# ErickRosete/tacorl

Hardware: NVIDIA B200
Metric: play_lmp_train_frames_per_sec (higher is better)
Workload: dtype bf16

## Files before the change

tacorl_b200/csrc/conv_tc.cu:

```cuda
#include "common.cuh"
#include "internal.h"
#include <cuda.h>
#include <cuda_bf16.h>
#include <algorithm>

namespace tacorl {

constexpr int CV_MAXT = 16;
constexpr int CV_STAGES = 8;
constexpr int CV_THREADS = 192;

struct ConvGeom {
  int BW, BH;
  int tiles_x, tiles_y, num_tiles;
  int ntaps;
  int tap_x[CV_MAXT], tap_p[CV_MAXT], tap_y[CV_MAXT];
  int RA, RB;
  int OH, OW, oys, oy0, oxs, ox0;
};

struct ConvEpi {
  const float* bias;
  int relu;
  const __nv_bfloat16* gate;
  __nv_bfloat16* out_bf16;
  float* out_f32;
};

__device__ __forceinline__ uint32_t cv_smem(const void* p) { return (uint32_t)__cvta_generic_to_shared(p); }
__device__ __forceinline__ void cv_mbar_init(uint32_t bar, uint32_t count) {
  asm volatile("mbarrier.init.shared::cta.b64 [%0], %1;" ::"r"(bar), "r"(count));
}
__device__ __forceinline__ void cv_mbar_expect_tx(uint32_t bar, uint32_t bytes) {
  asm volatile("mbarrier.arrive.expect_tx.shared::cta.b64 _, [%0], %1;" ::"r"(bar), "r"(bytes) : "memory");
}
__device__ __forceinline__ void cv_mbar_arrive(uint32_t bar) {
  asm volatile("mbarrier.arrive.shared::cta.b64 _, [%0];" ::"r"(bar) : "memory");
}
__device__ __forceinline__ void cv_mbar_wait(uint32_t bar, uint32_t parity) {
  uint32_t done;
  do {
    asm volatile(
        "{\n\t.reg .pred p;\n\t"
        "mbarrier.try_wait.parity.shared::cta.b64 p, [%1], %2;\n\t"
        "selp.u32 %0, 1, 0, p;\n\t}"
        : "=r"(done) : "r"(bar), "r"(parity) : "memory");
  } while (!done);
}
__device__ __forceinline__ void cv_tma_2d(uint32_t dst, const CUtensorMap* tm, int c0, int c1, uint32_t bar) {
  asm volatile(
      "cp.async.bulk.tensor.2d.shared::cluster.global.mbarrier::complete_tx::bytes [%0], [%1, {%2, %3}], [%4];"
      ::"r"(dst), "l"(tm), "r"(c0), "r"(c1), "r"(bar) : "memory");
}
__device__ __forceinline__ void cv_tma_4d(uint32_t dst, const CUtensorMap* tm, int c0, int c1, int c2, int c3, uint32_t bar) {
  asm volatile(
      "cp.async.bulk.tensor.4d.shared::cluster.global.mbarrier::complete_tx::bytes [%0], [%1, {%2, %3, %4, %5}], [%6];"
      ::"r"(dst), "l"(tm), "r"(c0), "r"(c1), "r"(c2), "r"(c3), "r"(bar) : "memory");
}
__device__ __forceinline__ void cv_tma_5d(uint32_t dst, const CUtensorMap* tm, int c0, int c1, int c2, int c3, int c4,
                                          uint32_t bar) {
  asm volatile(
      "cp.async.bulk.tensor.5d.shared::cluster.global.mbarrier::complete_tx::bytes [%0], [%1, {%2, %3, %4, %5, %6}], [%7];"
      ::"r"(dst), "l"(tm), "r"(c0), "r"(c1), "r"(c2), "r"(c3), "r"(c4), "r"(bar) : "memory");
}
__device__ __forceinline__ void cv_cp16(uint32_t dst, const void* src, uint32_t src_bytes) {
  asm volatile("cp.async.cg.shared.global [%0], [%1], 16, %2;" ::"r"(dst), "l"(src), "r"(src_bytes) : "memory");
}
__device__ __forceinline__ void cv_cp_async_arrive(uint32_t bar) {
  asm volatile("cp.async.mbarrier.arrive.noinc.shared::cta.b64 [%0];" ::"r"(bar) : "memory");
}
__device__ __forceinline__ void cv_st32(void* p, const uint32_t (&v)[8]) {
  asm volatile("st.global.v8.b32 [%0], {%1,%2,%3,%4,%5,%6,%7,%8};"
               ::"l"(p), "r"(v[0]), "r"(v[1]), "r"(v[2]), "r"(v[3]), "r"(v[4]), "r"(v[5]), "r"(v[6]), "r"(v[7]) : "memory");
}
__device__ __forceinline__ void cv_commit_group() { asm volatile("cp.async.commit_group;" ::: "memory"); }
template <int N> __device__ __forceinline__ void cv_wait_group() {
  asm volatile("cp.async.wait_group %0;" ::"n"(N) : "memory");
}
__device__ __forceinline__ void cv_wait_group_dyn(int n) {
  switch (n) {
    case 0: cv_wait_group<0>(); break;
    case 1: cv_wait_group<1>(); break;
    case 2: cv_wait_group<2>(); break;
    case 3: cv_wait_group<3>(); break;
    default: cv_wait_group<4>(); break;
  }
}
__device__ __forceinline__ void cv_fence_async() { asm volatile("fence.proxy.async.shared::cta;" ::: "memory"); }
__device__ __forceinline__ void cv_fence_before() { asm volatile("tcgen05.fence::before_thread_sync;" ::: "memory"); }
__device__ __forceinline__ void cv_fence_after() { asm volatile("tcgen05.fence::after_thread_sync;" ::: "memory"); }
__device__ __forceinline__ void cv_commit(uint32_t bar) {
  asm volatile("tcgen05.commit.cta_group::1.mbarrier::arrive::one.shared::cluster.b64 [%0];" ::"r"(bar) : "memory");
}
__device__ __forceinline__ void cv_mma(uint32_t tmem_d, uint64_t adesc, uint64_t bdesc, uint32_t idesc, uint32_t acc) {
  asm volatile(
      "{\n\t.reg .pred p;\n\t"
      "setp.ne.b32 p, %4, 0;\n\t"
      "tcgen05.mma.cta_group::1.kind::f16 [%0], %1, %2, %3, p;\n\t}"
      ::"r"(tmem_d), "l"(adesc), "l"(bdesc), "r"(idesc), "r"(acc) : "memory");
}
__device__ __forceinline__ void cv_ld16(uint32_t taddr, uint32_t (&r)[16]) {
  asm volatile(
      "tcgen05.ld.sync.aligned.32x32b.x16.b32 {%0,%1,%2,%3,%4,%5,%6,%7,%8,%9,%10,%11,%12,%13,%14,%15}, [%16];"
      : "=r"(r[0]), "=r"(r[1]), "=r"(r[2]), "=r"(r[3]), "=r"(r[4]), "=r"(r[5]), "=r"(r[6]), "=r"(r[7]),
        "=r"(r[8]), "=r"(r[9]), "=r"(r[10]), "=r"(r[11]), "=r"(r[12]), "=r"(r[13]), "=r"(r[14]), "=r"(r[15])
      : "r"(taddr));
  asm volatile("tcgen05.wait::ld.sync.aligned;" ::: "memory");
}
__device__ __forceinline__ void cv_ld16_nowait(uint32_t taddr, uint32_t (&r)[16]) {
  asm volatile(
      "tcgen05.ld.sync.aligned.32x32b.x16.b32 {%0,%1,%2,%3,%4,%5,%6,%7,%8,%9,%10,%11,%12,%13,%14,%15}, [%16];"
      : "=r"(r[0]), "=r"(r[1]), "=r"(r[2]), "=r"(r[3]), "=r"(r[4]), "=r"(r[5]), "=r"(r[6]), "=r"(r[7]),
        "=r"(r[8]), "=r"(r[9]), "=r"(r[10]), "=r"(r[11]), "=r"(r[12]), "=r"(r[13]), "=r"(r[14]), "=r"(r[15])
      : "r"(taddr));
}
__device__ __forceinline__ void cv_ld_wait() { asm volatile("tcgen05.wait::ld.sync.aligned;" ::: "memory"); }
__device__ __forceinline__ uint64_t cv_desc(uint32_t saddr, uint32_t lbo, uint32_t sbo) {
  uint64_t d = 0;
  d |= (uint64_t)((saddr >> 4) & 0x3FFF);
  d |= (uint64_t)((lbo >> 4) & 0x3FFF) << 16;
  d |= (uint64_t)((sbo >> 4) & 0x3FFF) << 32;
  d |= (uint64_t)1 << 46;
  d |= (uint64_t)2 << 61;
  return d;
}

// ... 37 lines not shown
  __syncthreads();
  cv_fence_after();
  const uint32_t tmem_base = *tmem_slot;

  if (warp == 0) {
    if (lane == 0) {
      cv_mbar_expect_tx(w_bar, g.ntaps * W_TAP_BYTES);
      for (int t = 0; t < g.ntaps; ++t) cv_tma_2d(w_base + t * W_TAP_BYTES, &tmW, 0, t * BN, w_bar);
      const uint32_t box_bytes = (uint32_t)(g.BW * g.BH) * 128;
      uint32_t it = 0;
      for (int tile = blockIdx.x; tile < g.num_tiles; tile += gridDim.x) {
        const int n = tile / tiles_per_frame, rem = tile - n * tiles_per_frame;
        const int ty = rem / g.tiles_x, tx = rem - ty * g.tiles_x;
        const int x0 = tx * g.BW, y0 = ty * g.BH;
        for (int t = 0; t < g.ntaps; ++t, ++it) {
          const int s = it % CV_STAGES;
          cv_mbar_wait(empty_bar(s), ((it / CV_STAGES) & 1) ^ 1);
          cv_mbar_expect_tx(full_bar(s), box_bytes);
          cv_tma_5d(a_base + s * A_BYTES, &tmA, 0, x0 + g.tap_x[t], g.tap_p[t], y0 + g.tap_y[t], n, full_bar(s));
        }
      }
    }
  } else if (warp == 1) {
    if (lane == 0) {
      cv_mbar_wait(w_bar, 0);
      const uint32_t idesc = (1u << 4) | (1u << 7) | (1u << 10) | ((uint32_t)(BN >> 3) << 17) | ((uint32_t)(128 >> 4) << 24);
      uint64_t bdesc[NTAPS * 4];
#pragma unroll
      for (int i = 0; i < NTAPS * 4; ++i) bdesc[i] = cv_desc(w_base + (i >> 2) * W_TAP_BYTES + (i & 3) * 32, 16, 1024);
      const uint64_t adesc0 = cv_desc(a_base, 16, 1024);
      uint32_t it = 0, lt = 0;
      for (int tile = blockIdx.x; tile < g.num_tiles; tile += gridDim.x, ++lt) {
        const uint32_t acc = lt & 1;
        cv_mbar_wait(tempty_bar(acc), ((lt >> 1) & 1) ^ 1);
        cv_fence_after();
        const uint32_t tmem_d = tmem_base + acc * ACC_COLS;
#pragma unroll
        for (int t = 0; t < NTAPS; ++t, ++it) {
          const int s = it % CV_STAGES;
          cv_mbar_wait(full_bar(s), (it / CV_STAGES) & 1);
          cv_fence_after();
          const uint64_t adesc = adesc0 + (uint64_t)(s * (A_BYTES >> 4));
#pragma unroll
          for (int k = 0; k < 4; ++k) cv_mma(tmem_d, adesc + 2 * k, bdesc[t * 4 + k], idesc, (t > 0 || k > 0) ? 1u : 0u);
          cv_commit(empty_bar(s));
        }
        cv_commit(tfull_bar(acc));
      }
    }
  } else {
    const int q = warp & 3;
    const int r = q * 32 + lane;
    const int a_l = r / g.BW, b_l = r - a_l * g.BW;
    uint32_t lt = 0;
    for (int tile = blockIdx.x; tile < g.num_tiles; tile += gridDim.x, ++lt) {
      const uint32_t acc = lt & 1;
      const int n = tile / tiles_per_frame, rem = tile - n * tiles_per_frame;
      const int ty = rem / g.tiles_x, tx = rem - ty * g.tiles_x;
      const int a = ty * g.BH + a_l, b = tx * g.BW + b_l;
      const bool row_ok = a_l < g.BH && a < g.RA && b < g.RB;
      const long long opix = row_ok ? ((long long)n * g.OH + (a * g.oys + g.oy0)) * g.OW + (b * g.oxs + g.ox0) : 0;
      uint4 gate[BN / 8];
      if (ep.gate && row_ok) {
        const uint4* gp = reinterpret_cast<const uint4*>(ep.gate + opix * BN);
#pragma unroll
        for (int j = 0; j < BN / 8; ++j) gate[j] = __ldg(gp + j);
      }
      cv_mbar_wait(tfull_bar(acc), (lt >> 1) & 1);
      cv_fence_after();
#pragma unroll
      for (int c0 = 0; c0 < BN; c0 += 16) {
        uint32_t rr[16];
        cv_ld16(tmem_base + acc * ACC_COLS + ((uint32_t)(q * 32) << 16) + c0, rr);
        if (!row_ok) continue;
        float v[16];
#pragma unroll
        for (int j = 0; j < 16; ++j) v[j] = __uint_as_float(rr[j]) + s_bias[c0 + j];
        if (ep.relu) {
#pragma unroll
          for (int j = 0; j < 16; ++j) v[j] = fmaxf(v[j], 0.f);
        }
        if (ep.gate) {
          const uint4 g0 = gate[c0 / 8], g1 = gate[c0 / 8 + 1];
          const __nv_bfloat162* h0 = reinterpret_cast<const __nv_bfloat162*>(&g0);
          const __nv_bfloat162* h1 = reinterpret_cast<const __nv_bfloat162*>(&g1);
#pragma unroll
          for (int j = 0; j < 4; ++j) {
            const float2 f0 = __bfloat1622float2(h0[j]), f1 = __bfloat1622float2(h1[j]);
            if (f0.x <= 0.f) v[2 * j] = 0.f;
            if (f0.y <= 0.f) v[2 * j + 1] = 0.f;
            if (f1.x <= 0.f) v[8 + 2 * j] = 0.f;
            if (f1.y <= 0.f) v[8 + 2 * j + 1] = 0.f;
          }
        }
        if (ep.out_bf16) {
          uint32_t pk[8];
#pragma unroll
          for (int j = 0; j < 8; ++j) {
            __nv_bfloat162 t2 = __floats2bfloat162_rn(v[2 * j], v[2 * j + 1]);
            pk[j] = *reinterpret_cast<uint32_t*>(&t2);
          }
          cv_st32(ep.out_bf16 + opix * BN + c0, pk);
        }
        if (ep.out_f32) {
          uint32_t lo[8], hi[8];
#pragma unroll
          for (int j = 0; j < 8; ++j) { lo[j] = __float_as_uint(v[j]); hi[j] = __float_as_uint(v[8 + j]); }
          cv_st32(ep.out_f32 + opix * BN + c0, lo);
          cv_st32(ep.out_f32 + opix * BN + c0 + 8, hi);
        }
      }
      cv_fence_before();
      __syncwarp();
      if (lane == 0) cv_mbar_arrive(tempty_bar(acc));
    }
  }
  cv_fence_before();
  __syncthreads();
  if (warp == 1) {
    cv_fence_after();
    asm volatile("tcgen05.dealloc.cta_group::1.sync.aligned.b32 %0, %1;" ::"r"(tmem_base), "r"(TMEM_COLS) : "memory");
  }
}

struct ConvLinGeom {
  int W, OH, OW;
  int frame_rows;
  int tiles_per_frame, num_tiles;
  int ntaps, load_rows;
  int stages;
  int shift[CV_MAXT];
  int OHt, OWt, oys, oy0, oxs, ox0;
};
constexpr int CL_MAX_STAGES = 8;

template <int BN, int NTAPS, int KSTEPS>
__global__ void __launch_bounds__(CV_THREADS, 1)
conv_lin_kernel(const __grid_constant__ ConvLinGeom g, const __grid_constant__ CUtensorMap tmA,
                const __grid_constant__ CUtensorMap tmW, const ConvEpi ep) {
  constexpr uint32_t W_TAP_BYTES = BN * 128;
  constexpr uint32_t ACC_COLS = BN < 32 ? 32 : BN;
  constexpr int NACC = 4;
  constexpr uint32_t TMEM_COLS = NACC * ACC_COLS;
  extern __shared__ __align__(1024) uint8_t smem_raw[];
  uint8_t* smem = (uint8_t*)(((uintptr_t)smem_raw + 1023) & ~(uintptr_t)1023);
  const uint32_t stage_bytes = ((uint32_t)g.load_rows * 128 + 1023) & ~1023u;
  const uint32_t w_base = cv_smem(smem);
  const uint32_t a_base = w_base + g.ntaps * W_TAP_BYTES;
  uint64_t* bars = (uint64_t*)(smem + g.ntaps * W_TAP_BYTES + g.stages * stage_bytes);
  const int CL_STAGES = g.stages;
  uint32_t* tmem_slot = (uint32_t*)(bars + 2 * CL_MAX_STAGES + 2 * NACC + 1);
  auto full_bar = [&](int s) { return cv_smem(bars + s); };
  auto empty_bar = [&](int s) { return cv_smem(bars + CL_MAX_STAGES + s); };
  auto tfull_bar = [&](int a) { return cv_smem(bars + 2 * CL_MAX_STAGES + a); };
  auto tempty_bar = [&](int a) { return cv_smem(bars + 2 * CL_MAX_STAGES + NACC + a); };
  const uint32_t w_bar = cv_smem(bars + 2 * CL_MAX_STAGES + 2 * NACC);
  const int warp = threadIdx.x >> 5, lane = threadIdx.x & 31;
  __shared__ float s_bias[BN];
  if (threadIdx.x < BN) s_bias[threadIdx.x] = ep.bias ? ep.bias[threadIdx.x] : 0.f;

  if (threadIdx.x == 0) {
    for (int s = 0; s < CL_STAGES; ++s) { cv_mbar_init(full_bar(s), 1); cv_mbar_init(empty_bar(s), 1); }
    for (int a = 0; a < NACC; ++a) { cv_mbar_init(tfull_bar(a), 1); cv_mbar_init(tempty_bar(a), 4); }
    cv_mbar_init(w_bar, 1);
    asm volatile("fence.mbarrier_init.release.cluster;" ::: "memory");
  }
  if (warp == 1) {
// ... 166 lines not shown
  __syncthreads();
  cv_fence_after();
  const uint32_t tmem_base = *tmem_slot;

  if (warp == 0) {
    if (lane == 0) {
      cv_mbar_expect_tx(w_bar, 4 * W_TAP_BYTES);
      for (int t = 0; t < 4; ++t) cv_tma_2d(w_base + t * W_TAP_BYTES, &tmW, 0, t * 128, w_bar);
      uint32_t it = 0;
      for (int tile = blockIdx.x; tile < g.num_tiles; tile += gridDim.x, ++it) {
        const int n = tile / tiles_per_frame, rem = tile - n * tiles_per_frame;
        const int ty = rem / g.tiles_x, tx = rem - ty * g.tiles_x;
        const int s = it % DG_STAGES;
        cv_mbar_wait(empty_bar(s), ((it / DG_STAGES) & 1) ^ 1);
        cv_mbar_expect_tx(full_bar(s), A_BYTES);
        cv_tma_4d(a_base + s * A_BYTES, &tmA, 0, tx * (DG_PW - 1) - 1, ty * (DG_PH - 1) - 1, n, full_bar(s));
      }
    }
  } else if (warp == 1) {
    if (lane == 0) {
      cv_mbar_wait(w_bar, 0);
      const uint32_t idesc = (1u << 4) | (1u << 7) | (1u << 10) | ((uint32_t)(128 >> 3) << 17) | ((uint32_t)(128 >> 4) << 24);
      uint32_t aoff[16];
      uint64_t bdesc[16];
#pragma unroll
      for (int t = 0; t < 4; ++t)
#pragma unroll
        for (int k = 0; k < 4; ++k) {
          const int j = t >> 1, i = t & 1;
          aoff[t * 4 + k] = (uint32_t)(((1 - j) * DG_PW + (1 - i)) * 128 + k * 32) >> 4;
          bdesc[t * 4 + k] = cv_desc(w_base + t * W_TAP_BYTES + k * 32, 16, 1024);
        }
      const uint64_t adesc0 = cv_desc(a_base, 16, 1024);
      uint32_t it = 0;
      for (int tile = blockIdx.x; tile < g.num_tiles; tile += gridDim.x, ++it) {
        const uint32_t acc = it & 1;
        const int s = it % DG_STAGES;
        cv_mbar_wait(tempty_bar(acc), ((it >> 1) & 1) ^ 1);
        cv_mbar_wait(full_bar(s), (it / DG_STAGES) & 1);
        cv_fence_after();
        const uint32_t tmem_d = tmem_base + acc * ACC_COLS;
        const uint64_t adesc = adesc0 + (uint64_t)(s * (A_BYTES >> 4));
#pragma unroll
        for (int i = 0; i < 16; ++i) cv_mma(tmem_d, adesc + aoff[i], bdesc[i], idesc, i > 0 ? 1u : 0u);
        cv_commit(empty_bar(s));
        cv_commit(tfull_bar(acc));
      }
    }
  } else {
    const int q = warp & 3;
    const int half = (warp - 2) >> 2;
    const int r = q * 32 + lane;
    const int al = r / DG_PW, bl = r - al * DG_PW;
    uint32_t lt = 0;
    for (int tile = blockIdx.x; tile < g.num_tiles; tile += gridDim.x, ++lt) {
      const uint32_t acc = lt & 1;
      const int n = tile / tiles_per_frame, rem = tile - n * tiles_per_frame;
      const int ty = rem / g.tiles_x, tx = rem - ty * g.tiles_x;
      const int a = ty * (DG_PH - 1) + al, b = tx * (DG_PW - 1) + bl;
      const bool row_ok = al < DG_PH - 1 && bl < DG_PW - 1 && a < g.RA && b < g.RB;
      bool okc[2];
      long long opixc[2], dpixc[2];
      uint4 gate[2][4];
#pragma unroll
      for (int c2 = 0; c2 < 2; ++c2) {
        const int oy = 2 * a + half, ox = 2 * b + c2;
        okc[c2] = row_ok && oy < g.H1 && ox < g.W1;
        opixc[c2] = okc[c2] ? ((long long)n * g.H1 + oy) * g.W1 + ox : 0;
        dpixc[c2] = okc[c2] ? ((long long)n * g.OHp + oy) * g.OWp + ox : 0;
        const uint4* gp = reinterpret_cast<const uint4*>(y1 + opixc[c2] * 32);
#pragma unroll
        for (int j = 0; j < 4; ++j) gate[c2][j] = __ldg(gp + j);
      }
      cv_mbar_wait(tfull_bar(acc), (lt >> 1) & 1);
      cv_fence_after();
#pragma unroll
      for (int c2 = 0; c2 < 2; ++c2) {
        const int cls = 2 * half + c2;
        const bool ok = okc[c2];
        const long long opix = dpixc[c2];
        uint32_t r2[2][16];
        cv_ld16_nowait(tmem_base + acc * ACC_COLS + ((uint32_t)(q * 32) << 16) + cls * 32, r2[0]);
        cv_ld16_nowait(tmem_base + acc * ACC_COLS + ((uint32_t)(q * 32) << 16) + cls * 32 + 16, r2[1]);
        cv_ld_wait();
#pragma unroll
        for (int c0 = 0; c0 < 32; c0 += 16) {
          const uint32_t (&rr)[16] = r2[c0 / 16];
          if (!ok) continue;
          const uint4 g0 = gate[c2][c0 / 8], g1 = gate[c2][c0 / 8 + 1];
          const __nv_bfloat162* h0 = reinterpret_cast<const __nv_bfloat162*>(&g0);
          const __nv_bfloat162* h1 = reinterpret_cast<const __nv_bfloat162*>(&g1);
          float v[16];
#pragma unroll
          for (int j = 0; j < 16; ++j) v[j] = __uint_as_float(rr[j]);
#pragma unroll
          for (int j = 0; j < 4; ++j) {
            const float2 f0 = __bfloat1622float2(h0[j]), f1 = __bfloat1622float2(h1[j]);
            if (f0.x <= 0.f) v[2 * j] = 0.f;
            if (f0.y <= 0.f) v[2 * j + 1] = 0.f;
            if (f1.x <= 0.f) v[8 + 2 * j] = 0.f;
            if (f1.y <= 0.f) v[8 + 2 * j + 1] = 0.f;
          }
          uint32_t pk[8];
#pragma unroll
          for (int j = 0; j < 8; ++j) {
            __nv_bfloat162 t2 = __floats2bfloat162_rn(v[2 * j], v[2 * j + 1]);
            pk[j] = *reinterpret_cast<uint32_t*>(&t2);
          }
          cv_st32(dy1 + opix * 32 + c0, pk);
        }
      }
      cv_fence_before();
      __syncwarp();
      if (lane == 0) cv_mbar_arrive(tempty_bar(acc));
    }
  }
  cv_fence_before();
  __syncthreads();
  if (warp == 1) {
    cv_fence_after();
    asm volatile("tcgen05.dealloc.cta_group::1.sync.aligned.b32 %0, %1;" ::"r"(tmem_base), "r"(TMEM_COLS) : "memory");
  }
}

typedef CUresult (*CvEncodeFn)(CUtensorMap*, CUtensorMapDataType, cuuint32_t, void*, const cuuint64_t*,
                               const cuuint64_t*, const cuuint32_t*, const cuuint32_t*, CUtensorMapInterleave,
                               CUtensorMapSwizzle, CUtensorMapL2promotion, CUtensorMapFloatOOBfill);
static CvEncodeFn cv_encode_fn() {
  static CvEncodeFn fn = nullptr;
  if (!fn) {
    void* p = nullptr;
    cudaDriverEntryPointQueryResult q;
    if (cudaGetDriverEntryPoint("cuTensorMapEncodeTiled", &p, cudaEnableDefault, &q) == cudaSuccess &&
        q == cudaDriverEntryPointSuccess)
      fn = (CvEncodeFn)p;
  }
  return fn;
}

static int cv_weight_tmap(CUtensorMap* tm, const void* wp, int ntaps, int BN) {
  CvEncodeFn fn = cv_encode_fn();
  TACORL_REQUIRE(fn, "conv_tc: cuTensorMapEncodeTiled is not available");
  TACORL_REQUIRE(((uintptr_t)wp & 15) == 0, "conv_tc: packed weights must be 16-byte aligned");
  cuuint64_t dims[2] = {64, (cuuint64_t)ntaps * BN};
  cuuint64_t strides[1] = {128};
  cuuint32_t box[2] = {64, (cuuint32_t)BN};
  cuuint32_t estr[2] = {1, 1};
  CUresult r = fn(tm, CU_TENSOR_MAP_DATA_TYPE_BFLOAT16, 2, const_cast<void*>(wp), dims, strides, box, estr,
                  CU_TENSOR_MAP_INTERLEAVE_NONE, CU_TENSOR_MAP_SWIZZLE_128B, CU_TENSOR_MAP_L2_PROMOTION_L2_256B,
                  CU_TENSOR_MAP_FLOAT_OOB_FILL_NONE);
  TACORL_REQUIRE(r == CUDA_SUCCESS, "conv_tc: cuTensorMapEncodeTiled(weights) failed (%d)", (int)r);
  return 0;
}

struct ActView {
  const void* base;
  long long nx, np, ny, nn;
  long long sx, sp, sy, sn;
};
static int cv_act_tmap(CUtensorMap* tm, const ActView& v, int BW, int BH) {
  CvEncodeFn fn = cv_encode_fn();
  TACORL_REQUIRE(fn, "conv_tc: cuTensorMapEncodeTiled is not available");
  TACORL_REQUIRE(((uintptr_t)v.base & 15) == 0 && v.sx % 16 == 0 && v.sp % 16 == 0 && v.sy % 16 == 0 && v.sn % 16 == 0,
                 "conv_tc: activation view must be 16-byte aligned (strides %lld %lld %lld %lld)", v.sx, v.sp, v.sy, v.sn);
  cuuint64_t dims[5] = {64, (cuuint64_t)v.nx, (cuuint64_t)v.np, (cuuint64_t)v.ny, (cuuint64_t)v.nn};
  cuuint64_t strides[4] = {(cuuint64_t)v.sx, (cuuint64_t)v.sp, (cuuint64_t)v.sy, (cuuint64_t)v.sn};
  cuuint32_t box[5] = {64, (cuuint32_t)BW, 1, (cuuint32_t)BH, 1};
  cuuint32_t estr[5] = {1, 1, 1, 1, 1};
  CUresult r = fn(tm, CU_TENSOR_MAP_DATA_TYPE_BFLOAT16, 5, const_cast<void*>(v.base), dims, strides, box, estr,
                  CU_TENSOR_MAP_INTERLEAVE_NONE, CU_TENSOR_MAP_SWIZZLE_128B, CU_TENSOR_MAP_L2_PROMOTION_L2_256B,
                  CU_TENSOR_MAP_FLOAT_OOB_FILL_NONE);
  TACORL_REQUIRE(r == CUDA_SUCCESS, "conv_tc: cuTensorMapEncodeTiled(activation) failed (%d): dims %lld %lld %lld %lld box %dx%d",
                 (int)r, v.nx, v.np, v.ny, v.nn, BW, BH);
  return 0;
}

static void cv_choose_patch(int RA, int RB, int* BW, int* BH) {
  long long best = -1;
  *BW = 1; *BH = 1;
  for (int bw = 1; bw <= 128 && bw <= RB; ++bw)
    for (int bh = 1; bh * bw <= 128 && bh <= RA; ++bh) {
      const long long tiles = (long long)cdiv(RB, bw) * cdiv(RA, bh);
      const long long score = -tiles * 1024 + bw;
      if (best == -1 || score > best) { best = score; *BW = bw; *BH = bh; }
    }
}

template <int BN, int NTAPS>
static int cv_launch(const ConvGeom& g, const ActView& view, const void* wpacked, const ConvEpi& ep, cudaStream_t st) {
  CUtensorMap tw, ta;
  int rc = cv_weight_tmap(&tw, wpacked, g.ntaps, BN);
  if (rc) return rc;
  if ((rc = cv_act_tmap(&ta, view, g.BW, g.BH))) return rc;
  const size_t smem = (size_t)g.ntaps * BN * 128 + CV_STAGES * 128 * 128 + (2 * CV_STAGES + 5) * 8 + 16 + 1024;
  static size_t configured = 0;
  auto kern = conv_tc_kernel<BN, NTAPS>;
  if (smem > configured) {
    TACORL_CHECK_CUDA(cudaFuncSetAttribute(kern, cudaFuncAttributeMaxDynamicSharedMemorySize, (int)smem));
    configured = smem;
  }
  const int ctas = g.num_tiles < persistent_ctas() ? g.num_tiles : persistent_ctas();
  kern<<<ctas, CV_THREADS, smem, st>>>(g, ta, tw, ep);
  TACORL_LAUNCH_CHECK();
  return 0;
}

static int conv_tc_run(ConvGeom g, int N, const ActView& view, int BN, const void* wpacked, const ConvEpi& ep,
                       cudaStream_t st) {
  if (N == 0 || g.RA <= 0 || g.RB <= 0) return 0;
  TACORL_REQUIRE(g.ntaps >= 1 && g.ntaps <= CV_MAXT, "conv_tc: bad tap count %d", g.ntaps);
  cv_choose_patch(g.RA, g.RB, &g.BW, &g.BH);
  g.tiles_x = cdiv(g.RB, g.BW); g.tiles_y = cdiv(g.RA, g.BH);
  g.num_tiles = N * g.tiles_x * g.tiles_y;
  if (BN == 32 && g.ntaps == 4) return cv_launch<32, 4>(g, view, wpacked, ep, st);
  if (BN == 64 && g.ntaps == 8) return cv_launch<64, 8>(g, view, wpacked, ep, st);
  if (BN == 64 && g.ntaps == 9) return cv_launch<64, 9>(g, view, wpacked, ep, st);
  set_last_error("conv_tc: unsupported output width %d / tap count %d", BN, g.ntaps);
  return -1;
}

template <int BN, int NTAPS, int KSTEPS>
static int cl_launch(ConvLinGeom g, int N, const void* src, const void* wpacked, const ConvEpi& ep, cudaStream_t st) {
  CvEncodeFn fn = cv_encode_fn();
  TACORL_REQUIRE(fn, "conv_lin: cuTensorMapEncodeTiled is not available");
  int max_shift = 0;
  for (int t = 0; t < g.ntaps; ++t) max_shift = g.shift[t] > max_shift ? g.shift[t] : max_shift;
  g.load_rows = (128 + max_shift + 7) & ~7;
  TACORL_REQUIRE(g.load_rows <= 256, "conv_lin: input window of %d pixel rows exceeds one TMA box", g.load_rows);
  const int lin = (g.OH - 1) * g.W + g.OW;
  g.tiles_per_frame = cdiv(lin, 128);
  g.num_tiles = N * g.tiles_per_frame;
  CUtensorMap tw, ta;
  int rc = cv_weight_tmap(&tw, wpacked, g.ntaps, BN);
  if (rc) return rc;
  {
    TACORL_REQUIRE(((uintptr_t)src & 15) == 0, "conv_lin: activation must be 16-byte aligned");
    cuuint64_t dims[2] = {64, (cuuint64_t)N * g.frame_rows};
    cuuint64_t strides[1] = {128};
    cuuint32_t box[2] = {64, (cuuint32_t)g.load_rows};
    cuuint32_t estr[2] = {1, 1};
    CUresult r = fn(&ta, CU_TENSOR_MAP_DATA_TYPE_BFLOAT16, 2, const_cast<void*>(src), dims, strides, box, estr,
                    CU_TENSOR_MAP_INTERLEAVE_NONE, CU_TENSOR_MAP_SWIZZLE_128B, CU_TENSOR_MAP_L2_PROMOTION_L2_256B,
                    CU_TENSOR_MAP_FLOAT_OOB_FILL_NONE);
    TACORL_REQUIRE(r == CUDA_SUCCESS, "conv_lin: cuTensorMapEncodeTiled(activation) failed (%d)", (int)r);
  }
  const size_t stage = ((size_t)g.load_rows * 128 + 1023) & ~(size_t)1023;
  const size_t fixed = (size_t)g.ntaps * BN * 128 + (2 * CL_MAX_STAGES + 12) * 8 + 16 + 1024 + 256;
  g.stages = (int)std::min<size_t>(CL_MAX_STAGES, (227 * 1024 - fixed) / stage);
  TACORL_REQUIRE(g.stages >= 2, "conv_lin: input window of %zu bytes leaves no room for a stage ring", stage);
  const size_t smem = fixed - 256 + g.stages * stage;
  static size_t configured = 0;
  TACORL_REQUIRE(g.ntaps == NTAPS, "conv_lin: tap count mismatch");
  auto kern = conv_lin_kernel<BN, NTAPS, KSTEPS>;
  if (smem > configured) {
    TACORL_CHECK_CUDA(cudaFuncSetAttribute(kern, cudaFuncAttributeMaxDynamicSharedMemorySize, (int)smem));
    configured = smem;
  }
  const int ctas = g.num_tiles < persistent_ctas() ? g.num_tiles : persistent_ctas();
  kern<<<ctas, CV_THREADS, smem, st>>>(g, ta, tw, ep);
  TACORL_LAUNCH_CHECK();
  return 0;
}

int conv_lin_conv3_fwd(const void* y2b, int N, int H2, int W2, int H3, int W3, const void* wp, const float* bias,
                       float* y3, cudaStream_t st) {
  if (128 + 2 * W2 + 2 > 256)
    return conv_tc_conv3_fwd(y2b, N, H2, W2, H3, W3, wp, bias, y3, st);
  ConvLinGeom g = {};
  g.W = W2; g.OH = H3; g.OW = W3; g.frame_rows = H2 * W2; g.ntaps = 9;
  for (int t = 0; t < 9; ++t) g.shift[t] = (t / 3) * W2 + (t % 3);
  g.OHt = H3; g.OWt = W3; g.oys = 1; g.oxs = 1;
  ConvEpi e = {bias, 1, nullptr, nullptr, y3};
  return cl_launch<64, 9, 4>(g, N, y2b, wp, e, st);
}
int conv_lin_conv1_fwd(const void* xs, int N, int H1, int W1, const void* wp, const float* bias, void* y1b,
                       cudaStream_t st) {
  if (128 + (W1 + 1) + 1 > 256)
    return conv_tc_conv1_fwd(xs, N, H1, W1, wp, bias, y1b, st);
  ConvLinGeom g = {};
  g.W = W1 + 1; g.OH = H1; g.OW = W1; g.frame_rows = (H1 + 1) * (W1 + 1); g.ntaps = 4;
  for (int t = 0; t < 4; ++t) g.shift[t] = (t >> 1) * (W1 + 1) + (t & 1);
  g.OHt = H1; g.OWt = W1; g.oys = 1; g.oxs = 1;
  ConvEpi e = {bias, 1, nullptr, (__nv_bfloat16*)y1b, nullptr};
  return cl_launch<32, 4, 3>(g, N, xs, wp, e, st);
}

__global__ void cv_zero_margin_kernel(uint4* __restrict__ t, int N, int H, int W, int Hp, int Wp, int chunks) {
  const int right = H * (Wp - W), all = right + (Hp - H) * Wp;
  const long long total = (long long)N * all * chunks;
  for (long long i = blockIdx.x * (long long)blockDim.x + threadIdx.x; i < total; i += (long long)gridDim.x * blockDim.x) {
    const int c = (int)(i % chunks);
    const long long r = i / chunks;
    const int m = (int)(r % all);
    const long long n = r / all;
    const int pp = m < right ? (m / (Wp - W)) * Wp + W + m % (Wp - W) : H * Wp + (m - right);
    t[(n * Hp * Wp + pp) * chunks + c] = make_uint4(0, 0, 0, 0);
  }
}

int conv_dgrad2_fused(const void* dy2b, int N, int H1, int W1, int H2, int W2, const void* wp5, const void* y1b, void* dy1b,
                      int out_pad, cudaStream_t st) {
  if (N == 0) return 0;
  CvEncodeFn fn = cv_encode_fn();
  TACORL_REQUIRE(fn, "conv_dgrad2: cuTensorMapEncodeTiled is not available");
  Dgrad2Geom g = {};
  g.H1 = H1; g.W1 = W1; g.H2 = H2; g.W2 = W2; g.RA = (H1 + 1) / 2; g.RB = (W1 + 1) / 2;
  g.tiles_x = cdiv(g.RB, DG_PW - 1); g.tiles_y = cdiv(g.RA, DG_PH - 1);
  g.num_tiles = N * g.tiles_x * g.tiles_y;
  g.OHp = H1 + out_pad; g.OWp = W1 + out_pad;
  if (out_pad > 0) {
    const long long total = (long long)N * (H1 * out_pad + out_pad * g.OWp) * 4;
    cv_zero_margin_kernel<<<(int)min((long long)592, (total + 255) / 256), 256, 0, st>>>((uint4*)dy1b, N, H1, W1, g.OHp, g.OWp, 4);
    TACORL_LAUNCH_CHECK();
  }
  CUtensorMap tw, ta;
  int rc = cv_weight_tmap(&tw, wp5, 4, 128);
  if (rc) return rc;
  {
    TACORL_REQUIRE(((uintptr_t)dy2b & 15) == 0, "conv_dgrad2: dy2 must be 16-byte aligned");
    cuuint64_t dims[4] = {64, (cuuint64_t)W2, (cuuint64_t)H2, (cuuint64_t)N};
    cuuint64_t strides[3] = {128, (cuuint64_t)W2 * 128, (cuuint64_t)H2 * W2 * 128};
    cuuint32_t box[4] = {64, DG_PW, DG_PH, 1};
    cuuint32_t estr[4] = {1, 1, 1, 1};
    CUresult r = fn(&ta, CU_TENSOR_MAP_DATA_TYPE_BFLOAT16, 4, const_cast<void*>(dy2b), dims, strides, box, estr,
                    CU_TENSOR_MAP_INTERLEAVE_NONE, CU_TENSOR_MAP_SWIZZLE_128B, CU_TENSOR_MAP_L2_PROMOTION_L2_256B,
                    CU_TENSOR_MAP_FLOAT_OOB_FILL_NONE);
    TACORL_REQUIRE(r == CUDA_SUCCESS, "conv_dgrad2: cuTensorMapEncodeTiled(dy2) failed (%d)", (int)r);
  }
  const size_t smem = 4 * 128 * 128 + (size_t)(DG_STAGES + 1) * 128 * 128 + (2 * DG_STAGES + 5) * 8 + 16 + 1024;
  static bool configured = false;
  if (!configured) {
    TACORL_CHECK_CUDA(cudaFuncSetAttribute(conv_dgrad2_kernel, cudaFuncAttributeMaxDynamicSharedMemorySize, (int)smem));
    configured = true;
  }
  const int ctas = g.num_tiles < persistent_ctas() ? g.num_tiles : persistent_ctas();
  conv_dgrad2_kernel<<<ctas, DG_THREADS, smem, st>>>(g, ta, tw, (const __nv_bfloat16*)y1b, (__nv_bfloat16*)dy1b);
  TACORL_LAUNCH_CHECK();
  return 0;
}

struct PackJobs {
  int n;
  int mode[3];
  const float* W[3];
  __nv_bfloat16* Wp[3];
  int total[3];
};
__global__ void cv_pack_kernel(const PackJobs jobs) {
  const int job = blockIdx.y;
  const int mode = jobs.mode[job], total = jobs.total[job];
  const float* __restrict__ W = jobs.W[job];
  __nv_bfloat16* __restrict__ Wp = jobs.Wp[job];
  const int i = blockIdx.x * blockDim.x + threadIdx.x;
  if (i >= total) return;
  const int k = i & 63;
  float v = 0.f;
  if (mode == 0) {
    const int oc = (i >> 6) & 63, t = i >> 12, ky = t / 3, kx = t % 3;
    v = W[((oc * 64 + k) * 3 + ky) * 3 + kx];
  } else if (mode == 1) {
    const int oc = (i >> 6) & 63, t = i >> 12, ky = t >> 1, p = t & 1, kx = 2 * p + (k >> 5), c = k & 31;
    v = W[((oc * 32 + c) * 4 + ky) * 4 + kx];
  } else if (mode == 2) {
    const int oc = (i >> 6) & 31, t = i >> 11, dy = t >> 1, dx = t & 1;
    if (k < 48) {
      const int c = k % 3, pp = k / 3, py = pp >> 2, px = pp & 3;
      v = W[((oc * 3 + c) * 8 + (4 * dy + py)) * 8 + (4 * dx + px)];
    }
  } else if (mode == 3) {
    const int c = (i >> 6) & 63, t = i >> 12, ky = t / 3, kx = t % 3;
    v = W[((k * 64 + c) * 3 + ky) * 3 + kx];
  } else if (mode == 4) {
// ... 10 lines not shown
  static const int totals[6] = {9 * 64 * 64, 8 * 64 * 64, 4 * 32 * 64, 9 * 64 * 64, 16 * 32 * 64, 4 * 128 * 64};
  TACORL_REQUIRE(n >= 1 && n <= 3, "conv_tc_pack: 1..3 tensors per launch");
  PackJobs jobs;
  jobs.n = n;
  int most = 0;
  for (int j = 0; j < n; ++j) {
    TACORL_REQUIRE(modes[j] >= 0 && modes[j] < 6, "conv_tc_pack: bad mode");
    jobs.mode[j] = modes[j]; jobs.W[j] = Ws[j]; jobs.Wp[j] = (__nv_bfloat16*)Wps[j]; jobs.total[j] = totals[modes[j]];
    most = max(most, totals[modes[j]]);
  }
  cv_pack_kernel<<<dim3(cdiv(most, 256), n), 256, 0, st>>>(jobs);
  TACORL_LAUNCH_CHECK();
  return 0;
}

int conv_tc_pack(int mode, const float* W, void* Wp, cudaStream_t st) {
  return conv_tc_pack_multi(1, &mode, &W, &Wp, st);
}

__global__ void cv_s2d_kernel(const float* __restrict__ x, int H, int W, int SH, int SW, long long total,
                              __nv_bfloat16* __restrict__ xs) {
  for (long long i = blockIdx.x * (long long)blockDim.x + threadIdx.x; i < total;
       i += (long long)gridDim.x * blockDim.x) {
    const int py = (int)(i & 3);
    long long t = i >> 2;
    const int X = (int)(t % SW); t /= SW;
    const int Y = (int)(t % SH);
    const long long n = t / SH;
    const int iy = 4 * Y + py;
    float4 c0 = make_float4(0, 0, 0, 0), c1 = c0, c2 = c0;
    if (iy < H && 4 * X + 3 < W) {
      const float* p = x + ((n * 3) * H + iy) * (long long)W + 4 * X;
      c0 = __ldg(reinterpret_cast<const float4*>(p));
      c1 = __ldg(reinterpret_cast<const float4*>(p + (long long)H * W));
      c2 = __ldg(reinterpret_cast<const float4*>(p + 2LL * H * W));
    }
    __nv_bfloat16* o = xs + ((n * SH + Y) * (long long)SW + X) * 64 + py * 12;
    if (py == 0) {
      reinterpret_cast<uint4*>(o + 48)[0] = make_uint4(0, 0, 0, 0);
      reinterpret_cast<uint4*>(o + 48)[1] = make_uint4(0, 0, 0, 0);
    }
    const float v[12] = {c0.x, c1.x, c2.x, c0.y, c1.y, c2.y, c0.z, c1.z, c2.z, c0.w, c1.w, c2.w};
    uint32_t pk[6];
#pragma unroll
    for (int j = 0; j < 6; ++j) {
      __nv_bfloat162 t2 = __floats2bfloat162_rn(v[2 * j], v[2 * j + 1]);
      pk[j] = *reinterpret_cast<uint32_t*>(&t2);
    }
    uint2* op = reinterpret_cast<uint2*>(o);
    op[0] = make_uint2(pk[0], pk[1]); op[1] = make_uint2(pk[2], pk[3]); op[2] = make_uint2(pk[4], pk[5]);
  }
}

__global__ void cv_s2d_u8_kernel(const unsigned char* __restrict__ x, int H, int W, int SH, int SW, long long total,
                                 float scale, float shift, __nv_bfloat16* __restrict__ xs) {
  for (long long i = blockIdx.x * (long long)blockDim.x + threadIdx.x; i < total;
       i += (long long)gridDim.x * blockDim.x) {
    const int py = (int)(i & 3);
    long long t = i >> 2;
    const int X = (int)(t % SW); t /= SW;
    const int Y = (int)(t % SH);
    const long long n = t / SH;
    const int iy = 4 * Y + py;
    float v[12];
#pragma unroll
    for (int j = 0; j < 12; ++j) v[j] = 0.f;
    if (iy < H && 4 * X + 3 < W) {
      const unsigned char* p = x + ((n * 3) * H + iy) * (long long)W + 4 * X;
#pragma unroll
      for (int c = 0; c < 3; ++c) {
        const uchar4 u = __ldg(reinterpret_cast<const uchar4*>(p + (long long)c * H * W));
        v[c] = fmaf((float)u.x, scale, shift); v[3 + c] = fmaf((float)u.y, scale, shift);
        v[6 + c] = fmaf((float)u.z, scale, shift); v[9 + c] = fmaf((float)u.w, scale, shift);
      }
    }
    __nv_bfloat16* o = xs + ((n * SH + Y) * (long long)SW + X) * 64 + py * 12;
    if (py == 0) {
      reinterpret_cast<uint4*>(o + 48)[0] = make_uint4(0, 0, 0, 0);
      reinterpret_cast<uint4*>(o + 48)[1] = make_uint4(0, 0, 0, 0);
    }
    uint32_t pk[6];
#pragma unroll
    for (int j = 0; j < 6; ++j) {
      __nv_bfloat162 t2 = __floats2bfloat162_rn(v[2 * j], v[2 * j + 1]);
      pk[j] = *reinterpret_cast<uint32_t*>(&t2);
    }
    uint2* op = reinterpret_cast<uint2*>(o);
    op[0] = make_uint2(pk[0], pk[1]); op[1] = make_uint2(pk[2], pk[3]); op[2] = make_uint2(pk[4], pk[5]);
  }
}

int conv_tc_s2d_u8(const unsigned char* x, int N, int H, int W, int SH, int SW, float scale, float shift, void* xs,
                   cudaStream_t st) {
  TACORL_REQUIRE(W % 4 == 0 && ((uintptr_t)x & 3) == 0, "conv_tc_s2d_u8: image width must be a multiple of 4");
  const long long total = (long long)N * SH * SW * 4;
  if (total == 0) return 0;
  cv_s2d_u8_kernel<<<(int)min((long long)148 * 16, (total + 255) / 256), 256, 0, st>>>(x, H, W, SH, SW, total, scale,
                                                                                     shift, (__nv_bfloat16*)xs);
  TACORL_LAUNCH_CHECK();
  return 0;
}

__global__ void cv_u8_to_f32_kernel(long long n, const unsigned char* __restrict__ x, float scale, float shift,
                                    float* __restrict__ o) {
  for (long long i = blockIdx.x * (long long)blockDim.x + threadIdx.x; i < n; i += (long long)gridDim.x * blockDim.x)
    o[i] = fmaf((float)x[i], scale, shift);
}

int u8_to_f32_normalized(long long n, const unsigned char* x, float scale, float shift, float* out, cudaStream_t st) {
  if (n == 0) return 0;
  cv_u8_to_f32_kernel<<<(int)min((long long)148 * 16, (n + 255) / 256), 256, 0, st>>>(n, x, scale, shift, out);
  TACORL_LAUNCH_CHECK();
  return 0;
}

int conv_tc_s2d(const float* x, int N, int H, int W, int SH, int SW, void* xs, cudaStream_t st) {
  TACORL_REQUIRE(W % 4 == 0 && ((uintptr_t)x & 15) == 0, "conv_tc_s2d: image width must be a multiple of 4");
  const long long total = (long long)N * SH * SW * 4;
  if (total == 0) return 0;
  cv_s2d_kernel<<<(int)min((long long)148 * 16, (total + 255) / 256), 256, 0, st>>>(x, H, W, SH, SW, total,
                                                                                  (__nv_bfloat16*)xs);
  TACORL_LAUNCH_CHECK();
  return 0;
}

static ActView cv_plain_view(const void* base, int N, int H, int W) {
  return ActView{base, W, 1, H, N, 128, 128, (long long)W * 128, (long long)H * W * 128};
}
int conv_tc_conv1_fwd(const void* xs, int N, int H1, int W1, const void* wp, const float* bias, void* y1b,
                      cudaStream_t st) {
  ConvGeom g = {};
  g.RA = H1; g.RB = W1; g.ntaps = 4;
  for (int t = 0; t < 4; ++t) { g.tap_y[t] = t >> 1; g.tap_x[t] = t & 1; }
  g.OH = H1; g.OW = W1; g.oys = 1; g.oxs = 1;
  ConvEpi e = {bias, 1, nullptr, (__nv_bfloat16*)y1b, nullptr};
  return conv_tc_run(g, N, cv_plain_view(xs, N, H1 + 1, W1 + 1), 32, wp, e, st);
}
int conv_tc_conv2_fwd(const void* y1b, int N, int H1, int W1, int H2, int W2, const void* wp, const float* bias,
                      void* y2b, cudaStream_t st) {
  ConvGeom g = {};
  g.RA = H2; g.RB = W2; g.ntaps = 8;
  for (int t = 0; t < 8; ++t) { const int ky = t >> 1; g.tap_x[t] = t & 1; g.tap_p[t] = ky & 1; g.tap_y[t] = ky >> 1; }
  g.OH = H2; g.OW = W2; g.oys = 1; g.oxs = 1;
  ConvEpi e = {bias, 1, nullptr, (__nv_bfloat16*)y2b, nullptr};
  const ActView v{y1b, W2 + 1, 2, H2 + 1, N, 128, (long long)W1 * 64, (long long)W1 * 128, (long long)H1 * W1 * 64};
  return conv_tc_run(g, N, v, 64, wp, e, st);
}
int conv_tc_conv3_fwd(const void* y2b, int N, int H2, int W2, int H3, int W3, const void* wp, const float* bias,
                      float* y3, cudaStream_t st) {
  ConvGeom g = {};
  g.RA = H3; g.RB = W3; g.ntaps = 9;
// ... 767 lines not shown
```

Before: 328,000.

## Prefetch gates a tile ahead, fuse margin zeroing, and restage s2d stores

The conv epilogue now prefetches the ReLU gate for the next tile with 32-byte non-coherent loads, overlapping that load with the wait on the current accumulator. The dgrad2 epilogue covers the padded output region and writes zeros for the margin itself, which removes the separate margin-zeroing kernel launch. The u8 space-to-depth kernel now has one thread handle a whole pixel, converts bytes to float with a bit trick, and stages results in swizzled shared memory so the warp writes coalesced 16-byte stores. New alignment requirements are added, and the prefetch holds more registers in flight.

New measurement: 333,700, median of 6. 1.02x the previous value.

```diff
diff --git a/tacorl_b200/csrc/conv_tc.cu b/tacorl_b200/csrc/conv_tc.cu
--- a/tacorl_b200/csrc/conv_tc.cu
+++ b/tacorl_b200/csrc/conv_tc.cu
@@ -72,6 +72,13 @@
 __device__ __forceinline__ void cv_st32(void* p, const uint32_t (&v)[8]) {
   asm volatile("st.global.v8.b32 [%0], {%1,%2,%3,%4,%5,%6,%7,%8};"
                ::"l"(p), "r"(v[0]), "r"(v[1]), "r"(v[2]), "r"(v[3]), "r"(v[4]), "r"(v[5]), "r"(v[6]), "r"(v[7]) : "memory");
+}
+__device__ __forceinline__ uint4 cv_ld32_nc(const void* p, uint4& hi) {
+  uint4 lo;
+  asm volatile("ld.global.nc.v8.b32 {%0,%1,%2,%3,%4,%5,%6,%7}, [%8];"
+               : "=r"(lo.x), "=r"(lo.y), "=r"(lo.z), "=r"(lo.w), "=r"(hi.x), "=r"(hi.y), "=r"(hi.z), "=r"(hi.w)
+               : "l"(p));
+  return lo;
 }
 __device__ __forceinline__ void cv_commit_group() { asm volatile("cp.async.commit_group;" ::: "memory"); }
 template <int N> __device__ __forceinline__ void cv_wait_group() {
@@ -215,20 +222,29 @@
     const int q = warp & 3;
     const int r = q * 32 + lane;
     const int a_l = r / g.BW, b_l = r - a_l * g.BW;
-    uint32_t lt = 0;
-    for (int tile = blockIdx.x; tile < g.num_tiles; tile += gridDim.x, ++lt) {
-      const uint32_t acc = lt & 1;
+    struct Row { bool ok; long long opix; };
+    auto row_of = [&](int tile) {
       const int n = tile / tiles_per_frame, rem = tile - n * tiles_per_frame;
       const int ty = rem / g.tiles_x, tx = rem - ty * g.tiles_x;
       const int a = ty * g.BH + a_l, b = tx * g.BW + b_l;
-      const bool row_ok = a_l < g.BH && a < g.RA && b < g.RB;
-      const long long opix = row_ok ? ((long long)n * g.OH + (a * g.oys + g.oy0)) * g.OW + (b * g.oxs + g.ox0) : 0;
-      uint4 gate[BN / 8];
-      if (ep.gate && row_ok) {
-        const uint4* gp = reinterpret_cast<const uint4*>(ep.gate + opix * BN);
-#pragma unroll
-        for (int j = 0; j < BN / 8; ++j) gate[j] = __ldg(gp + j);
-      }
+      Row w;
+      w.ok = a_l < g.BH && a < g.RA && b < g.RB;
+      w.opix = w.ok ? ((long long)n * g.OH + (a * g.oys + g.oy0)) * g.OW + (b * g.oxs + g.ox0) : 0;
+      return w;
+    };
+    auto load_gate = [&](int tile, uint4 (&gate)[BN / 8]) {
+      if (!ep.gate || tile >= g.num_tiles) return;
+      const Row w = row_of(tile);
+      if (!w.ok) return;
+#pragma unroll
+      for (int j = 0; j < BN / 8; j += 2) gate[j] = cv_ld32_nc(ep.gate + w.opix * BN + j * 8, gate[j + 1]);
+    };
+    auto drain = [&](int tile, uint32_t lt, const uint4 (&gate)[BN / 8], uint4 (&next)[BN / 8]) {
+      load_gate(tile + gridDim.x, next);
+      const uint32_t acc = lt & 1;
+      const Row w = row_of(tile);
+      const bool row_ok = w.ok;
+      const long long opix = w.opix;
       cv_mbar_wait(tfull_bar(acc), (lt >> 1) & 1);
       cv_fence_after();
 #pragma unroll
@@ -276,6 +292,13 @@
       cv_fence_before();
       __syncwarp();
       if (lane == 0) cv_mbar_arrive(tempty_bar(acc));
+    };
+    uint4 ga[BN / 8], gb[BN / 8];
+    load_gate(blockIdx.x, ga);
+    uint32_t lt = 0;
+    for (int tile = blockIdx.x; tile < g.num_tiles; tile += 2 * gridDim.x, lt += 2) {
+      drain(tile, lt, ga, gb);
+      if (tile + (int)gridDim.x < g.num_tiles) drain(tile + gridDim.x, lt + 1, gb, ga);
     }
   }
   cv_fence_before();
@@ -548,33 +571,40 @@
     const int half = (warp - 2) >> 2;
     const int r = q * 32 + lane;
     const int al = r / DG_PW, bl = r - al * DG_PW;
+    struct Pix { long long n; int oy, ox; bool frame, inner; };
+    auto pixel = [&](int tile, int c2) {
+      Pix p;
+      p.n = tile / tiles_per_frame;
+      const int rem = tile - (int)p.n * tiles_per_frame;
+      const int ty = rem / g.tiles_x, tx = rem - ty * g.tiles_x;
+      const int a = ty * (DG_PH - 1) + al, b = tx * (DG_PW - 1) + bl;
+      p.oy = 2 * a + half; p.ox = 2 * b + c2;
+      p.frame = al < DG_PH - 1 && bl < DG_PW - 1 && a < g.RA && b < g.RB && p.oy < g.OHp && p.ox < g.OWp;
+      p.inner = p.frame && p.oy < g.H1 && p.ox < g.W1;
+      return p;
+    };
+    auto load_gates = [&](int tile, uint4 (&gate)[2][4]) {
+#pragma unroll
+      for (int c2 = 0; c2 < 2; ++c2) {
+        const Pix p = pixel(tile, c2);
+        const long long gpix = p.inner ? (p.n * g.H1 + p.oy) * g.W1 + p.ox : 0;
+        gate[c2][0] = cv_ld32_nc(y1 + gpix * 32, gate[c2][1]);
+        gate[c2][2] = cv_ld32_nc(y1 + gpix * 32 + 16, gate[c2][3]);
+      }
+    };
     uint32_t lt = 0;
     for (int tile = blockIdx.x; tile < g.num_tiles; tile += gridDim.x, ++lt) {
       const uint32_t acc = lt & 1;
-      const int n = tile / tiles_per_frame, rem = tile - n * tiles_per_frame;
-      const int ty = rem / g.tiles_x, tx = rem - ty * g.tiles_x;
-      const int a = ty * (DG_PH - 1) + al, b = tx * (DG_PW - 1) + bl;
-      const bool row_ok = al < DG_PH - 1 && bl < DG_PW - 1 && a < g.RA && b < g.RB;
-      bool okc[2];
-      long long opixc[2], dpixc[2];
       uint4 gate[2][4];
-#pragma unroll
-      for (int c2 = 0; c2 < 2; ++c2) {
-        const int oy = 2 * a + half, ox = 2 * b + c2;
-        okc[c2] = row_ok && oy < g.H1 && ox < g.W1;
-        opixc[c2] = okc[c2] ? ((long long)n * g.H1 + oy) * g.W1 + ox : 0;
-        dpixc[c2] = okc[c2] ? ((long long)n * g.OHp + oy) * g.OWp + ox : 0;
-        const uint4* gp = reinterpret_cast<const uint4*>(y1 + opixc[c2] * 32);
-#pragma unroll
-        for (int j = 0; j < 4; ++j) gate[c2][j] = __ldg(gp + j);
-      }
+      load_gates(tile, gate);
       cv_mbar_wait(tfull_bar(acc), (lt >> 1) & 1);
       cv_fence_after();
 #pragma unroll
       for (int c2 = 0; c2 < 2; ++c2) {
         const int cls = 2 * half + c2;
-        const bool ok = okc[c2];
-        const long long opix = dpixc[c2];
+        const Pix p = pixel(tile, c2);
+        const bool ok = p.inner;
+        const long long opix = p.frame ? (p.n * g.OHp + p.oy) * g.OWp + p.ox : 0;
         uint32_t r2[2][16];
         cv_ld16_nowait(tmem_base + acc * ACC_COLS + ((uint32_t)(q * 32) << 16) + cls * 32, r2[0]);
         cv_ld16_nowait(tmem_base + acc * ACC_COLS + ((uint32_t)(q * 32) << 16) + cls * 32 + 16, r2[1]);
@@ -582,6 +612,10 @@
 #pragma unroll
         for (int c0 = 0; c0 < 32; c0 += 16) {
           const uint32_t (&rr)[16] = r2[c0 / 16];
+          if (p.frame && !ok) {
+            const uint32_t zero[8] = {0, 0, 0, 0, 0, 0, 0, 0};
+            cv_st32(dy1 + opix * 32 + c0, zero);
+          }
           if (!ok) continue;
           const uint4 g0 = gate[c2][c0 / 8], g1 = gate[c2][c0 / 8 + 1];
           const __nv_bfloat162* h0 = reinterpret_cast<const __nv_bfloat162*>(&g0);
@@ -684,6 +718,7 @@
 
 template <int BN, int NTAPS>
 static int cv_launch(const ConvGeom& g, const ActView& view, const void* wpacked, const ConvEpi& ep, cudaStream_t st) {
+  TACORL_REQUIRE(((uintptr_t)ep.gate & 31) == 0, "conv_tc: ReLU gate must be 32-byte aligned");
   CUtensorMap tw, ta;
   int rc = cv_weight_tmap(&tw, wpacked, g.ntaps, BN);
   if (rc) return rc;
@@ -781,39 +816,23 @@
   return cl_launch<32, 4, 3>(g, N, xs, wp, e, st);
 }
 
-__global__ void cv_zero_margin_kernel(uint4* __restrict__ t, int N, int H, int W, int Hp, int Wp, int chunks) {
-  const int right = H * (Wp - W), all = right + (Hp - H) * Wp;
-  const long long total = (long long)N * all * chunks;
-  for (long long i = blockIdx.x * (long long)blockDim.x + threadIdx.x; i < total; i += (long long)gridDim.x * blockDim.x) {
-    const int c = (int)(i % chunks);
-    const long long r = i / chunks;
-    const int m = (int)(r % all);
-    const long long n = r / all;
-    const int pp = m < right ? (m / (Wp - W)) * Wp + W + m % (Wp - W) : H * Wp + (m - right);
-    t[(n * Hp * Wp + pp) * chunks + c] = make_uint4(0, 0, 0, 0);
-  }
-}
-
 int conv_dgrad2_fused(const void* dy2b, int N, int H1, int W1, int H2, int W2, const void* wp5, const void* y1b, void* dy1b,
                       int out_pad, cudaStream_t st) {
   if (N == 0) return 0;
   CvEncodeFn fn = cv_encode_fn();
   TACORL_REQUIRE(fn, "conv_dgrad2: cuTensorMapEncodeTiled is not available");
   Dgrad2Geom g = {};
-  g.H1 = H1; g.W1 = W1; g.H2 = H2; g.W2 = W2; g.RA = (H1 + 1) / 2; g.RB = (W1 + 1) / 2;
+  g.H1 = H1; g.W1 = W1; g.H2 = H2; g.W2 = W2;
+  g.OHp = H1 + out_pad; g.OWp = W1 + out_pad;
+  g.RA = (g.OHp + 1) / 2; g.RB = (g.OWp + 1) / 2;
   g.tiles_x = cdiv(g.RB, DG_PW - 1); g.tiles_y = cdiv(g.RA, DG_PH - 1);
   g.num_tiles = N * g.tiles_x * g.tiles_y;
-  g.OHp = H1 + out_pad; g.OWp = W1 + out_pad;
-  if (out_pad > 0) {
-    const long long total = (long long)N * (H1 * out_pad + out_pad * g.OWp) * 4;
-    cv_zero_margin_kernel<<<(int)min((long long)592, (total + 255) / 256), 256, 0, st>>>((uint4*)dy1b, N, H1, W1, g.OHp, g.OWp, 4);
-    TACORL_LAUNCH_CHECK();
-  }
   CUtensorMap tw, ta;
   int rc = cv_weight_tmap(&tw, wp5, 4, 128);
   if (rc) return rc;
   {
     TACORL_REQUIRE(((uintptr_t)dy2b & 15) == 0, "conv_dgrad2: dy2 must be 16-byte aligned");
+    TACORL_REQUIRE(((uintptr_t)y1b & 31) == 0, "conv_dgrad2: y1 must be 32-byte aligned");
     cuuint64_t dims[4] = {64, (cuuint64_t)W2, (cuuint64_t)H2, (cuuint64_t)N};
     cuuint64_t strides[3] = {128, (cuuint64_t)W2 * 128, (cuuint64_t)H2 * W2 * 128};
     cuuint32_t box[4] = {64, DG_PW, DG_PH, 1};
@@ -930,51 +949,70 @@
   }
 }
 
-__global__ void cv_s2d_u8_kernel(const unsigned char* __restrict__ x, int H, int W, int SH, int SW, long long total,
-                                 float scale, float shift, __nv_bfloat16* __restrict__ xs) {
-  for (long long i = blockIdx.x * (long long)blockDim.x + threadIdx.x; i < total;
-       i += (long long)gridDim.x * blockDim.x) {
-    const int py = (int)(i & 3);
-    long long t = i >> 2;
-    const int X = (int)(t % SW); t /= SW;
-    const int Y = (int)(t % SH);
-    const long long n = t / SH;
-    const int iy = 4 * Y + py;
-    float v[12];
-#pragma unroll
-    for (int j = 0; j < 12; ++j) v[j] = 0.f;
-    if (iy < H && 4 * X + 3 < W) {
-      const unsigned char* p = x + ((n * 3) * H + iy) * (long long)W + 4 * X;
-#pragma unroll
-      for (int c = 0; c < 3; ++c) {
-        const uchar4 u = __ldg(reinterpret_cast<const uchar4*>(p + (long long)c * H * W));
-        v[c] = fmaf((float)u.x, scale, shift); v[3 + c] = fmaf((float)u.y, scale, shift);
-        v[6 + c] = fmaf((float)u.z, scale, shift); v[9 + c] = fmaf((float)u.w, scale, shift);
-      }
-    }
-    __nv_bfloat16* o = xs + ((n * SH + Y) * (long long)SW + X) * 64 + py * 12;
-    if (py == 0) {
-      reinterpret_cast<uint4*>(o + 48)[0] = make_uint4(0, 0, 0, 0);
-      reinterpret_cast<uint4*>(o + 48)[1] = make_uint4(0, 0, 0, 0);
-    }
-    uint32_t pk[6];
-#pragma unroll
-    for (int j = 0; j < 6; ++j) {
-      __nv_bfloat162 t2 = __floats2bfloat162_rn(v[2 * j], v[2 * j + 1]);
-      pk[j] = *reinterpret_cast<uint32_t*>(&t2);
-    }
-    uint2* op = reinterpret_cast<uint2*>(o);
-    op[0] = make_uint2(pk[0], pk[1]); op[1] = make_uint2(pk[2], pk[3]); op[2] = make_uint2(pk[4], pk[5]);
+constexpr int S2D_THREADS = 256;
+__global__ void __launch_bounds__(S2D_THREADS, 5) cv_s2d_u8_kernel(const unsigned char* __restrict__ x, int H, int W,
+                                                                int SH, int SW, long long total, float scale,
+                                                                float shift, uint4* __restrict__ xs) {
+  __shared__ uint4 stage[S2D_THREADS / 32][32 * 8];
+  const int lane = threadIdx.x & 31;
+  uint4* sw = stage[threadIdx.x >> 5];
+  for (long long base = blockIdx.x * (long long)blockDim.x + (threadIdx.x & ~31); base < total;
+       base += (long long)gridDim.x * blockDim.x) {
+    const long long i = base + lane;
+    if (i < total) {
+      const long long n = i / ((long long)SH * SW);
+      const int rem = (int)(i - n * SH * SW), Y = rem / SW, X = rem - Y * SW;
+      uint32_t u[4][3];
+      bool ok[4];
+#pragma unroll
+      for (int py = 0; py < 4; ++py) {
+        const int iy = 4 * Y + py;
+        ok[py] = iy < H && 4 * X + 3 < W;
+        const unsigned char* p = x + ((n * 3) * H + (ok[py] ? iy : 0)) * (long long)W + (ok[py] ? 4 * X : 0);
+#pragma unroll
+        for (int c = 0; c < 3; ++c)
+          u[py][c] = ok[py] ? __ldg(reinterpret_cast<const unsigned int*>(p + (long long)c * H * W)) : 0u;
+      }
+      uint32_t pk[24];
+#pragma unroll
+      for (int py = 0; py < 4; ++py) {
+        float v[12];
+#pragma unroll
+        for (int px = 0; px < 4; ++px)
+#pragma unroll
+          for (int c = 0; c < 3; ++c)
+            v[px * 3 + c] = ok[py] ? fmaf(__uint_as_float(0x4B000000u | ((u[py][c] >> (8 * px)) & 0xFFu)) - 8388608.f,
+                                          scale, shift) : 0.f;
+#pragma unroll
+        for (int j = 0; j < 6; ++j) {
+          __nv_bfloat162 t2 = __floats2bfloat162_rn(v[2 * j], v[2 * j + 1]);
+          pk[py * 6 + j] = *reinterpret_cast<uint32_t*>(&t2);
+        }
+      }
+#pragma unroll
+      for (int j = 0; j < 6; ++j) sw[lane * 8 + (j ^ (lane & 7))] = make_uint4(pk[4 * j], pk[4 * j + 1], pk[4 * j + 2], pk[4 * j + 3]);
+      sw[lane * 8 + (6 ^ (lane & 7))] = make_uint4(0, 0, 0, 0);
+      sw[lane * 8 + (7 ^ (lane & 7))] = make_uint4(0, 0, 0, 0);
+    }
+    __syncwarp();
+    uint4* o = xs + base * 8;
+#pragma unroll
+    for (int k = 0; k < 8; ++k) {
+      const int e = k * 32 + lane, p = e >> 3;
+      if (base + p < total) o[e] = sw[p * 8 + ((e & 7) ^ (p & 7))];
+    }
+    __syncwarp();
   }
 }
 
 int conv_tc_s2d_u8(const unsigned char* x, int N, int H, int W, int SH, int SW, float scale, float shift, void* xs,
                    cudaStream_t st) {
   TACORL_REQUIRE(W % 4 == 0 && ((uintptr_t)x & 3) == 0, "conv_tc_s2d_u8: image width must be a multiple of 4");
-  const long long total = (long long)N * SH * SW * 4;
+  TACORL_REQUIRE(((uintptr_t)xs & 15) == 0, "conv_tc_s2d_u8: xs must be 16-byte aligned");
+  const long long total = (long long)N * SH * SW;
   if (total == 0) return 0;
-  cv_s2d_u8_kernel<<<(int)min((long long)148 * 16, (total + 255) / 256), 256, 0, st>>>(x, H, W, SH, SW, total, scale,
-                                                                                     shift, (__nv_bfloat16*)xs);
+  const long long blocks = std::min<long long>(5LL * persistent_ctas(), (total + S2D_THREADS - 1) / S2D_THREADS);
+  cv_s2d_u8_kernel<<<(int)blocks, S2D_THREADS, 0, st>>>(x, H, W, SH, SW, total, scale, shift, (uint4*)xs);
   TACORL_LAUNCH_CHECK();
   return 0;
 }
```
